# hila-chefer/Transformer-Explainability

Measured on AMD Instinct MI355X. Metric: relevance maps/sec (ViT-B/16 224^2, batch 64 per GPU, generate_LRP transformer_attribution), higher is better.
Workload: dtype f32 (3xbf16 split operands, 6 products, fp32 accumulate)

## Files before the change

### include/te_relprop.h

```cpp
#ifndef TE_RELPROP_H
#define TE_RELPROP_H

#include <stddef.h>
#include <stdint.h>

#ifdef __cplusplus
extern "C" {
#endif

typedef void* te_stream_t;
typedef uint16_t te_bf16_t;

enum {
  TE_OK = 0,
  TE_ERR_INVALID_ARG = -1,
  TE_ERR_WORKSPACE = -2,
  TE_ERR_UNSUPPORTED = -3,
  TE_ERR_NO_DEVICE = -4
};

enum { TE_VARIANT_OURS = 0, TE_VARIANT_LRP = 1, TE_IMPL_SIMPLE = 0x100 };

enum { TE_ROLLOUT_NORMALISE = 1, TE_ROLLOUT_CLS_FIXUP = 2, TE_ROLLOUT_ROW0 = 4 };

// ... 35 lines not shown
                             const float* q, int64_t q_sb, int64_t q_sh, int64_t q_sn,
                             const float* k, int64_t k_sb, int64_t k_sh, int64_t k_sn,
                             const float* Z,
                             float* cam_q, int64_t cq_sb, int64_t cq_sh, int64_t cq_sn,
                             float* cam_k, int64_t ck_sb, int64_t ck_sh, int64_t ck_sn,
                             int64_t B, int64_t H, int64_t N, int64_t D, float out_scale, int variant,
                             void* ws, size_t ws_bytes, te_stream_t stream);

size_t te_add_relprop_workspace_bytes(int64_t B, int64_t n);
int te_add_relprop_f32(const float* R, const float* X0, const float* X1, float* out0, float* out1,
                       int64_t B, int64_t n, int64_t x1_batch_stride, int variant,
                       void* ws, size_t ws_bytes, te_stream_t stream);

size_t te_add_relprop_deferred_workspace_bytes(int64_t B, int64_t n);
int te_add_relprop_deferred_f32(const float* R, const float* X0, const float* X1, float* a, float* b, float* fac,
                                int64_t B, int64_t n, int64_t x1_batch_stride,
                                void* ws, size_t ws_bytes, te_stream_t stream);

size_t te_add_bcast_relprop_workspace_bytes(int64_t B, int64_t H, int64_t N);
int te_add_bcast_relprop_f32(const float* R, const float* X0, const float* mask, float* out0,
                             float* out1, int64_t B, int64_t H, int64_t N, int variant,
                             void* ws, size_t ws_bytes, te_stream_t stream);

int te_add_bcast_relprop_deferred_f32(const float* R, const float* X0, const float* mask, float* a, float* out1,
                                      float* fac, int64_t B, int64_t H, int64_t N,
                                      void* ws, size_t ws_bytes, te_stream_t stream);

int te_clone_relprop_f32(const float* R0, const float* R1, const float* R2, const float* X,
                         float* out, int64_t n, te_stream_t stream);

int te_clone_relprop_scaled_f32(const float* R0, const float* s0, int64_t s0_stride,
                                const float* R1, const float* s1, int64_t s1_stride,
                                const float* R2, const float* s2, int64_t s2_stride,
                                const float* X, float* out, int64_t B, int64_t n, te_stream_t stream);

int te_index_select_relprop_f32(const float* R, const float* X, float* out,
                                int64_t B, int64_t N, int64_t C, int64_t index, te_stream_t stream);

int te_gradcam_headmean_f32(const float* grad, const float* cam, float* out,
                            int64_t B, int64_t H, int64_t N, te_stream_t stream);

size_t te_rollout_workspace_bytes(int64_t L, int64_t B, int64_t N);
size_t te_rollout_row0_workspace_bytes(int64_t B, int64_t N);
int te_rollout_f32(const float* cams, int64_t L, int64_t start_layer, int64_t B, int64_t N,
                   int flags, float* joint, void* ws, size_t ws_bytes, te_stream_t stream);

#define TE_X6_TILE_AUTO 0
#define TE_X6_TILE_128 1
#define TE_X6_TILE_256 2
#define TE_X6_TILE_128x128 3
#define TE_X6_TEST_DROP_HANDOVER 0x200
#define TE_X6_WHOLE_TILES 0x10000
#define TE_X6_TEST_SMALL_GRID 0x4000
#define TE_X6_X_PLANES_SIGNED 0x20000
#define TE_X6_TILE_Z_SHIFT 10
#define TE_X6_TILE_C_SHIFT 12
#define TE_X6_PHASE_SPLIT 4
#define TE_X6_PHASE_Z 8
#define TE_X6_PHASE_C 16
#define TE_X6_PHASE_MASK 28
int te_linear_relprop_x6_supported(int64_t T, int64_t in_f, int64_t out_f);
size_t te_linear_relprop_x6_workspace_bytes(int64_t T, int64_t in_f, int64_t out_f);
size_t te_linear_x6_weight_planes_bytes(int64_t in_f, int64_t out_f);
size_t te_linear_x6_planes_bytes(int64_t rows, int64_t K);
int te_linear_x6_prepare_weights_f32(const float* W, int64_t in_f, int64_t out_f, void* planes, size_t planes_bytes,
                                     te_stream_t stream);
int te_linear_x6_split_abs_f32(const float* X, int64_t rows, int64_t K, void* planes, size_t planes_bytes,
                               te_stream_t stream);
int te_linear_relprop_x6_f32(const float* R, const float* r_scale, int64_t r_scale_stride, int64_t rows_per_sample,
                             const float* X, const float* W, const void* w_planes, const void* x_planes,
                             const float* Y, const float* bias, float* out,
                             int64_t T, int64_t in_f, int64_t out_f, int flags, unsigned* status, void* ws,
                             size_t ws_bytes, te_stream_t stream);
int te_linear_relprop_x6_check(const void* ws, int64_t T, int64_t in_f, int64_t out_f, te_stream_t stream);

int te_linear_relprop_x6_general_supported(int64_t T, int64_t in_f, int64_t out_f, int variant);
size_t te_linear_x6_weight_planes_lrp_bytes(int64_t in_f, int64_t out_f);
int te_linear_x6_prepare_weights_lrp_f32(const float* W, int64_t in_f, int64_t out_f, void* planes, size_t planes_bytes,
                                         te_stream_t stream);
size_t te_linear_relprop_x6_general_workspace_bytes(int64_t T, int64_t in_f, int64_t out_f, int variant);
int te_linear_relprop_x6_general_f32(const float* R, const float* r_scale, int64_t r_scale_stride, int64_t rows_per_sample,
                                     const float* X, const float* W, const void* w_planes, const void* w_planes_lrp,
                                     const void* x_abs_planes, const float* Y, const float* bias, float* out,
                                     int64_t T, int64_t in_f, int64_t out_f, float alpha, int variant, int flags,
                                     unsigned* status, void* ws, size_t ws_bytes, te_stream_t stream);

int te_gemm_x6_supported(int64_t T, int64_t K, int64_t M);
size_t te_gemm_x6_workspace_bytes(int64_t T, int64_t K, int64_t M);
int te_linear_x6_split_matrix_f32(const float* A, int64_t rows, int64_t K, int transposed, void* planes,
                                  size_t planes_bytes, te_stream_t stream);
int te_gemm_x6_f32(const float* X, const void* x_planes, const void* w_planes, const float* bias, float* out,
                   int64_t T, int64_t K, int64_t M, int flags, unsigned* status, void* ws, size_t ws_bytes,
                   te_stream_t stream);
int te_linear_x6_split_dual_f32(const float* A, int64_t rows, int64_t K, void* planes, void* planes_abs,
                                size_t planes_bytes, te_stream_t stream);
int te_gelu_backward_x6_planes_f32(const float* dy, const float* x, int64_t rows, int64_t K, void* planes,
                                   size_t planes_bytes, te_stream_t stream);
int te_gelu_forward_x6_planes_f32(const float* x, float* y, int64_t rows, int64_t K, void* planes, void* planes_abs,
                                  size_t planes_bytes, te_stream_t stream);

int te_attention_forward_supported(int64_t N, int64_t D);
int te_attention_forward_f32(const float* qkv, float* z_qk, float* attn, float* out, void* out_planes,
                             void* out_abs_planes, size_t planes_bytes, int64_t B, int64_t H, int64_t N, int64_t D,
                             float scale, te_stream_t stream);
int te_attention_backward_f32(const float* d_out, const float* out, const float* qkv, const float* attn, float* d_attn,
                              float* d_qkv, int64_t B, int64_t H, int64_t N, int64_t D, float scale, int need_qk,
                              te_stream_t stream);

int te_attention_strided_supported(int64_t N, int64_t D);
size_t te_attention_backward_strided_workspace_bytes(int64_t B, int64_t H, int64_t N);
int te_attention_forward_strided_f32(const float* q, int64_t q_sb, int64_t q_sh, int64_t q_sn,
                                     const float* k, int64_t k_sb, int64_t k_sh, int64_t k_sn,
                                     const float* v, int64_t v_sb, int64_t v_sh, int64_t v_sn,
                                     const float* mask, float* z_qk, float* x_scaled, float* attn,
                                     float* out, int64_t o_sb, int64_t o_sh, int64_t o_sn,
                                     int64_t B, int64_t H, int64_t N, int64_t D, float scale, te_stream_t stream);
int te_attention_backward_strided_f32(const float* d_out, int64_t do_sb, int64_t do_sh, int64_t do_sn,
                                      const float* out, int64_t o_sb, int64_t o_sh, int64_t o_sn,
                                      const float* q, int64_t q_sb, int64_t q_sh, int64_t q_sn,
                                      const float* k, int64_t k_sb, int64_t k_sh, int64_t k_sn,
                                      const float* v, int64_t v_sb, int64_t v_sh, int64_t v_sn,
                                      const float* attn, float* d_attn,
                                      float* d_q, int64_t dq_sb, int64_t dq_sh, int64_t dq_sn,
                                      float* d_k, int64_t dk_sb, int64_t dk_sh, int64_t dk_sn,
                                      float* d_v, int64_t dv_sb, int64_t dv_sh, int64_t dv_sn,
                                      int64_t B, int64_t H, int64_t N, int64_t D, float scale, int need_qk,
                                      void* ws, size_t ws_bytes, te_stream_t stream);
// ... 239 lines not shown
```

### transformer-explainability_amd/csrc/te_linear_x6.hip

```cpp
#include <algorithm>
#include <cmath>
#include <type_traits>

#include "te_x6.h"

namespace {

constexpr int kRB = 3 * kFrag;
constexpr int kMinFrag = 4;
constexpr int kSpinMillis = 250;
constexpr int kErrWord = 1023;


enum { MODE_Z = 0, MODE_C = 1, MODE_G = 2, MODE_ZI = 3, MODE_Z1 = 4, MODE_CI = 5, MODE_X = 6, MODE_ZS = 7 };

__device__ __forceinline__ float bf16_f32(unsigned b) { return __uint_as_float(b << 16); }

enum { OP_ABS = 0, OP_POS = 1, OP_NEG = 2, OP_ID = 3 };
template <int OP>
__device__ __forceinline__ float apply_op(float x) {
  if constexpr (OP == OP_ID) return x;
  if constexpr (OP == OP_ABS) return __int_as_float(__float_as_int(x) & 0x7fffffff);
  const int b = __float_as_int(x);
  if constexpr (OP == OP_POS) return __int_as_float(b > 0 ? b : 0);
  return __int_as_float(b < 0 ? b : 0);
}

template <int OP, bool TRANSPOSE>
__global__ __launch_bounds__(256) void split_kernel(const float* __restrict__ src, unsigned char* __restrict__ dst,
                                                    int64_t R, int64_t K, int group, int sign,
                                                    unsigned char* __restrict__ dst_abs = nullptr) {
  const int r = threadIdx.x & 31, sl = threadIdx.x >> 5;
  const int64_t rb = blockIdx.x;
  const int64_t ks = (int64_t)blockIdx.y * 8 + sl;
  const int64_t nks = K >> 4;
  if (ks >= nks) return;
  const int64_t row = rb * 32 + r;
  float v[16];
  if (row < R) {
    if constexpr (!TRANSPOSE) {
      const float* s = src + row * K + ks * 16;
#pragma unroll
      for (int c = 0; c < 4; ++c) {
        const f32x4 q = *reinterpret_cast<const f32x4*>(s + 4 * c);
#pragma unroll
        for (int e = 0; e < 4; ++e) v[4 * c + e] = q[e];
      }
    } else {
#pragma unroll
      for (int e = 0; e < 16; ++e) v[e] = src[(ks * 16 + e) * R + row];
    }
  } else {
#pragma unroll
    for (int e = 0; e < 16; ++e) v[e] = 0.0f;
  }
  unsigned p[8][3];
#pragma unroll
  for (int e = 0; e < 8; ++e) split3_pk(apply_op<OP>(v[2 * e]), apply_op<OP>(v[2 * e + 1]), p[e]);
  unsigned char* d = dst + ((rb * nks + ks) * group + sign * 3) * kFrag + r * 16;
#pragma unroll
  for (int q = 0; q < 3; ++q)
#pragma unroll
    for (int kh = 0; kh < 2; ++kh) {
      u32x4 w;
// ... 88 lines not shown
      p[e][0] &= 0x7fff7fffu;
      p[e][1] ^= m & (((p[e][1] & 0x7fff7fffu) + 0x7fff7fffu) & 0x80008000u);
      p[e][2] ^= m & (((p[e][2] & 0x7fff7fffu) + 0x7fff7fffu) & 0x80008000u);
    }
    store(dst_abs + ((rb * nks + ks) * 3) * kFrag + r * 16);
  }
}

__global__ __launch_bounds__(256) void zero_words_kernel(u32x4* __restrict__ p) {
  p[(size_t)blockIdx.x * 256 + threadIdx.x] = u32x4{0u, 0u, 0u, 0u};
}

__device__ __forceinline__ float exact_z(const float* __restrict__ x, const float* __restrict__ w, int64_t K) {
  float z1 = 0.0f, z2 = 0.0f;
  for (int64_t k = 0; k < K; ++k) {
    const float xv = x[k], wv = w[k];
    z1 = fmaf(fmaxf(xv, 0.0f), fmaxf(wv, 0.0f), z1);
    z2 = fmaf(fminf(xv, 0.0f), fminf(wv, 0.0f), z2);
  }
  return z1 + z2;
}

__device__ __forceinline__ float exact_zi(const float* __restrict__ x, const float* __restrict__ w, int64_t K) {
  float z1 = 0.0f, z2 = 0.0f;
  for (int64_t k = 0; k < K; ++k) {
    const float xv = x[k], wv = w[k];
    z1 = fmaf(fmaxf(xv, 0.0f), fminf(wv, 0.0f), z1);
    z2 = fmaf(fminf(xv, 0.0f), fmaxf(wv, 0.0f), z2);
  }
  return z1 + z2;
}

struct X6Params {
  const unsigned char* A;
  const unsigned char* B;
  int64_t a_group_stride;
  int64_t b_rb_stride;
  int nks;
  unsigned char pad0_[20];
  int ntm, ntn;
  int rows_w;
  int t_fast;
  int whole_tiles;
  int pad1_;
  int ncb;
  int64_t T;
  int in_f, out_f;
  float* partial;
  unsigned* flags;
  unsigned* status;
  long long spin_ticks;
  int drop_handover;
  int small_grid;
  int prefer_whole;
  const float* R;
  const float* Y;
  const float* bias;
  const float* X;
  const float* W;
  unsigned char* S;
  const float* rs;
  int64_t rs_stride;
  int rps;
  float* out;
  float scale;
  int accum;
  int x_sign;
};

#if defined(__HIP_DEVICE_COMPILE__)
#define X6_PASS4(a, b, c, d) asm volatile("" : "+v"(a), "+v"(b), "+v"(c), "+v"(d))
#else
#define X6_PASS4(a, b, c, d) (void)0
#endif

__device__ __forceinline__ void glds16(const unsigned char* src, unsigned char* lds_wave_base) {
  __builtin_amdgcn_global_load_lds((const __attribute__((address_space(1))) void*)src,
                                   (__attribute__((address_space(3))) void*)lds_wave_base, 16, 0, 0);
}

constexpr int kStages = 2;
template <int WM>
struct X6Geo {
  static constexpr int NWM = (WM == 1) ? 1 : 2, NWN = (WM == 0) ? 2 : 4, MI = (WM == 0) ? 2 : 4;
  static constexpr int NW = NWM * NWN, THREADS = 64 * NW, WPS = (WM == 0) ? 3 : 2;
  static constexpr int TM = NWM * MI * 32, TT = NWN * 64;
  static constexpr int NPA = 3 * NWM * MI, NPB = 3 * NWN * 2;
  static constexpr int ACC = MI * 2 * 16;
  static constexpr int MAX_SPX = (WM == 2) ? 32 : (WM == 1) ? 64 : 96;
};

template <int WM, int MODE>
struct X6Lds {
  using GEO = X6Geo<WM>;
  static constexpr bool STAGED = (MODE == MODE_Z || MODE == MODE_ZS || MODE == MODE_ZI || MODE == MODE_Z1) && GEO::MI == 4;
  static constexpr int STAGES = kStages * (GEO::NPA + GEO::NPB) * kFrag;
  static constexpr int MAIN = (STAGED && GEO::NW * 16384 > STAGES) ? GEO::NW * 16384 : STAGES;
  static constexpr int TOTAL = MAIN + GEO::NW * 512 + 16;
};

template <int WM, int MODE>
__global__ __launch_bounds__(X6Geo<WM>::THREADS, X6Geo<WM>::WPS) void x6_kernel(const X6Params p) {
  using GEO = X6Geo<WM>;
  constexpr int NW = GEO::NW, NWM = GEO::NWM, NWN = GEO::NWN, MI = GEO::MI;
  constexpr bool SGN = MODE == MODE_ZS;
  constexpr bool Z_ABS = MODE == MODE_Z || SGN;
  constexpr bool IS_Z = (Z_ABS || MODE == MODE_ZI || MODE == MODE_Z1);
  constexpr bool IS_C = (MODE == MODE_C || MODE == MODE_CI);
  constexpr int G = IS_C ? 6 : 3;
  constexpr int NPA = GEO::NPA, NPB = GEO::NPB;
  constexpr int NP = NPA + NPB;
  static_assert(NPA / 3 == NW, "each wave stages one weight-side block");
  constexpr int PBW = NPB / 3 / NW;
  constexpr int STAGE = NP * kFrag;
  constexpr int GROUPS = NPA / G;
  constexpr int LDS_MAIN = X6Lds<WM, MODE>::MAIN;
  extern __shared__ __attribute__((aligned(16))) unsigned char smem[];

  const int lane = threadIdx.x & 63;
  const int wave = __builtin_amdgcn_readfirstlane(threadIdx.x >> 6);
  const int wm = wave / NWN, wn = wave % NWN;
  const int lane16 = lane * 16;

  const int bid = blockIdx.x, spx = gridDim.x >> 3;
  const int xcd = bid & 7, slot = bid >> 3;
  const int nks = p.nks;
  const int tiles = p.ntm * p.ntn;
  const int tx0 = (int)((int64_t)tiles * xcd / 8), tx1 = (int)((int64_t)tiles * (xcd + 1) / 8);
  const int ntx = tx1 - tx0;
  const int64_t iters = (int64_t)ntx * nks;
  auto cut = [&](int s) -> int64_t {
    int64_t b = iters * s / spx;
    const int r = (int)(b % nks);
    if (p.whole_tiles) return (2 * r < nks) ? b - r : b + (nks - r);
    if (r < kMinFrag) b -= r;
    else if (nks - r < kMinFrag) b += nks - r;
    return b;
  };
  const int64_t ib = cut(slot), ie = cut(slot + 1);
  if (ib >= ie) return;
  const int f_tile = (int)(ib / nks), kb = (int)(ib - (int64_t)f_tile * nks);
  const int l_tile = (int)((ie - 1) / nks), ke = (int)(ie - (int64_t)l_tile * nks);
  const bool tail = kb > 0;
  const bool head = (ke < nks) && !(f_tile == l_tile && tail);
  const int full0 = tail ? f_tile + 1 : f_tile, full1 = (ke < nks) ? l_tile - 1 : l_tile;
  const int nseq = (head ? 1 : 0) + (full1 >= full0 ? full1 - full0 + 1 : 0) + (tail ? 1 : 0);

  float* my_part = p.partial + (size_t)bid * GEO::THREADS * GEO::ACC;
  const float* in_part = p.partial + (size_t)(bid - 8) * GEO::THREADS * GEO::ACC;

  for (int seq = 0; seq < nseq; ++seq) {
    int tile, k0, k1;
    if (head && seq == 0) {
      tile = l_tile, k0 = 0, k1 = ke;
    } else if (tail && seq == nseq - 1) {
      tile = f_tile, k0 = kb, k1 = (f_tile == l_tile) ? ke : nks;
    } else {
      tile = full0 + seq - (head ? 1 : 0), k0 = 0, k1 = nks;
    }
    tile += tx0;
    int tn, tm;
    if (p.t_fast) {
      tm = tile / p.ntn, tn = tile - tm * p.ntn;
    } else {
      tn = tile / p.ntm, tm = tile - tn * p.ntm;
    }

    const unsigned char* srcA;
    if constexpr (!IS_C)
      srcA = p.A + (int64_t)(tm * GROUPS + wave) * p.a_group_stride + (int64_t)k0 * kRB;
    else
      srcA = p.A + (int64_t)(tm * GROUPS + (wave >> 1)) * p.a_group_stride + (int64_t)k0 * (2 * kRB) + (wave & 1) * kRB;
    const unsigned char* srcB[PBW];
#pragma unroll
    for (int u = 0; u < PBW; ++u) {
      const int cb = min(tn * (GEO::TT / 32) + wave * PBW + u, p.ncb - 1);
      srcB[u] = p.B + (int64_t)cb * p.b_rb_stride + (int64_t)k0 * kRB;
    }
    unsigned char* const ldsA = smem + wave * kRB;
    unsigned char* const ldsB = smem + NPA * kFrag + wave * (PBW * kRB);
    u32x4 breg[SGN ? PBW : 1][3];
    auto stage_in = [&](int stg, int adv) __attribute__((always_inline)) {
      srcA += adv * (G * kFrag);
#pragma unroll
      for (int u = 0; u < PBW; ++u) srcB[u] += adv * kRB;
#pragma unroll
      for (int q = 0; q < 3; ++q) glds16(srcA + q * kFrag + lane16, ldsA + stg * STAGE + q * kFrag);
#pragma unroll
      for (int u = 0; u < PBW; ++u)
#pragma unroll
        for (int q = 0; q < 3; ++q) {
          if constexpr (SGN) breg[u][q] = *reinterpret_cast<const u32x4*>(srcB[u] + q * kFrag + lane16);
          else glds16(srcB[u] + q * kFrag + lane16, ldsB + stg * STAGE + (u * 3 + q) * kFrag);
        }
    };
    auto sign_and_store = [&](int stg) __attribute__((always_inline)) {
#pragma unroll
      for (int u = 0; u < (SGN ? PBW : 0); ++u) {
#pragma unroll
        for (int e = 0; e < 4; ++e) {
          const unsigned m = breg[u][0][e] & 0x80008000u;
          breg[u][0][e] &= 0x7fff7fffu;
          breg[u][1][e] ^= m;
          breg[u][2][e] ^= m;
        }
#pragma unroll
// ... 487 lines not shown
      bool live[2];
#pragma unroll
      for (int ni = 0; ni < 2; ++ni) {
        const int64_t t = ((int64_t)tn * (GEO::TT / 32) + wn * 2 + ni) * 32 + tc;
        live[ni] = t < p.T;
        tt[ni] = live[ni] ? t : p.T - 1;
#pragma unroll
        for (int il = 0; il < MI / 2; ++il) {
          const float* xr = p.X + tt[ni] * p.in_f + (tm * (NWM * MI / 2) + wm * (MI / 2) + il) * 32 + 4 * h;
#pragma unroll
          for (int g = 0; g < 4; ++g) x4[ni][il][g] = *reinterpret_cast<const f32x4*>(xr + 8 * g);
        }
      }
#pragma unroll
      for (int ni = 0; ni < 2; ++ni)
#pragma unroll
        for (int il = 0; il < MI / 2; ++il) {
          float* orow = p.out + tt[ni] * p.in_f + (tm * (NWM * MI / 2) + wm * (MI / 2) + il) * 32 + 4 * h;
#pragma unroll
          for (int g = 0; g < 4; ++g) {
            f32x4 o;
#pragma unroll
            for (int c = 0; c < 4; ++c) {
              const float xv = x4[ni][il][g][c];
              const float xp = fmaxf(xv, 0.0f), xn = fminf(xv, 0.0f);
              if constexpr (MODE == MODE_C)
                o[c] = p.scale * (xp * acc[2 * il][ni][4 * g + c] + xn * acc[2 * il + 1][ni][4 * g + c]);
              else
                o[c] = p.scale * (xp * acc[2 * il + 1][ni][4 * g + c] + xn * acc[2 * il][ni][4 * g + c]);
            }
            if constexpr (MODE == MODE_CI) {
              const f32x4 prev = *reinterpret_cast<const f32x4*>(orow + 8 * g);
#pragma unroll
              for (int c = 0; c < 4; ++c) o[c] = prev[c] + o[c];
            }
            if (live[ni]) *reinterpret_cast<f32x4*>(orow + 8 * g) = o;
          }
        }
    }
    __syncthreads();
  }
}

static_assert(sizeof(X6Params) == 248, "X6Params is the kernel-argument block of x6_kernel");
static_assert(offsetof(X6Params, ntm) == 56 && offsetof(X6Params, ncb) == 80 && offsetof(X6Params, T) == 88 &&
              offsetof(X6Params, partial) == 104 && offsetof(X6Params, R) == 152 && offsetof(X6Params, out) == 224,
              "a field of X6Params moved in the kernel arguments");

inline size_t planes_bytes(int64_t rows, int64_t K) {
  return (size_t)te_ceil_div(rows, 32) * 32 * (size_t)K * 6;
}
inline bool bad_k(int64_t K) { return K < 16 || K % 16; }
constexpr size_t kPartialBytes = (size_t)512 * 256 * 128 * 4;
constexpr double kWholeTileSlack = 1.15;
constexpr size_t kFlagBytes = 65536;
constexpr int kFlagWords = kFlagBytes / 4;
constexpr int kUsedFlagWords = kErrWord + 1;
constexpr int kRulePasses = 2;
constexpr int kGeneralPasses = 8;

struct X6Workspace {
  size_t x_stride, s, s_stride, partial, flags, total;
  unsigned char* x(void* ws, int set) const { return (unsigned char*)ws + set * x_stride; }
  unsigned char* sp(void* ws, int set) const { return (unsigned char*)ws + s + set * s_stride; }
  float* acc(void* ws) const { return (float*)((unsigned char*)ws + partial); }
  unsigned* flag_region(const void* ws, int pass) const { return (unsigned*)((unsigned char*)ws + flags) + (size_t)pass * kFlagWords; }
};
inline X6Workspace x6_workspace(int64_t T, int64_t K, int64_t M, int xsets, int ssets, int passes) {
  X6Workspace l;
  l.x_stride = te_align_up(planes_bytes(T, K), 256);
  l.s_stride = te_align_up(planes_bytes(T, M), 256);
  l.s = xsets * l.x_stride;
  l.partial = l.s + ssets * l.s_stride;
  l.flags = l.partial + kPartialBytes;
  l.total = l.flags + passes * kFlagBytes;
  return l;
}
inline X6Workspace gemm_workspace(int64_t T, int64_t K, int64_t M) { return x6_workspace(T, K, M, 1, 0, 1); }
inline X6Workspace rule_workspace(int64_t T, int64_t in_f, int64_t out_f) { return x6_workspace(T, in_f, out_f, 1, 1, kRulePasses); }
inline X6Workspace general_workspace(int64_t T, int64_t in_f, int64_t out_f) { return x6_workspace(T, in_f, out_f, 2, 2, kGeneralPasses); }

struct X6WeightPlanes { size_t c, total; };
inline X6WeightPlanes weight_planes(int64_t in_f, int64_t out_f) {
  const size_t c = te_align_up(planes_bytes(out_f, in_f), 256);
  return {c, c + te_align_up(2 * planes_bytes(in_f, out_f), 256)};
}
struct X6WeightPlanesLrp { size_t wn, wpT, wnT, total; };
inline X6WeightPlanesLrp weight_planes_lrp(int64_t in_f, int64_t out_f) {
  const size_t za = te_align_up(planes_bytes(out_f, in_f), 256), ca = te_align_up(planes_bytes(in_f, out_f), 256);
  return {za, 2 * za, 2 * za + ca, 2 * za + 2 * ca};
}

constexpr int kTileMask = TE_X6_TILE_128 | TE_X6_TILE_256 | TE_X6_TILE_128x128;
constexpr int kProductFlags = kTileMask | TE_X6_WHOLE_TILES | TE_X6_TEST_DROP_HANDOVER | TE_X6_TEST_SMALL_GRID;
constexpr int kRuleFlags = kProductFlags | TE_X6_PHASE_MASK | TE_X6_X_PLANES_SIGNED | (kTileMask << TE_X6_TILE_Z_SHIFT) | (kTileMask << TE_X6_TILE_C_SHIFT);

inline int pick_wm(int64_t in_f, int64_t out_f) {
  if (out_f % 256 == 0 && in_f % 128 == 0) return 2;
  if (out_f % 128 == 0 && in_f % 64 == 0) return 1;
  return 0;
}

inline long long spin_ticks_for_current_device() {
  static long long cached[64] = {};
  int dev = 0;
  if (hipGetDevice(&dev) != hipSuccess || dev < 0 || dev >= 64) dev = 0;
  if (cached[dev] == 0) {
    int khz = 0;
    if (hipDeviceGetAttribute(&khz, hipDeviceAttributeWallClockRate, dev) != hipSuccess || khz <= 0) khz = 100000;
    cached[dev] = (long long)khz * kSpinMillis;
  }
  return cached[dev];
}

template <int WM, int MODE>
int launch_x6(const X6Params& p, hipStream_t stream) {
  using GEO = X6Geo<WM>;
  constexpr int lds = X6Lds<WM, MODE>::TOTAL;
  static_assert(lds * (WM == 0 ? 3 : WM == 1 ? 2 : 1) <= 160 * 1024, "LDS of the workgroups of one CU");
  static_assert((size_t)8 * GEO::MAX_SPX * GEO::THREADS * GEO::ACC * 4 <= kPartialBytes && 8 * GEO::MAX_SPX < kErrWord, "workspace");
  auto kern = x6_kernel<WM, MODE>;
  hipError_t e = hipFuncSetAttribute(reinterpret_cast<const void*>(kern), hipFuncAttributeMaxDynamicSharedMemorySize, lds);
  if (e != hipSuccess) return (int)e;
  X6Params q = p;
  q.ntm = p.rows_w / GEO::TM;
  q.ntn = (int)te_ceil_div(p.T, GEO::TT);
  const int64_t tiles = (int64_t)q.ntm * q.ntn;
  const int max_spx = p.small_grid ? 2 : GEO::MAX_SPX;
  const int spx = (int)std::min<int64_t>(max_spx, std::max<int64_t>(1, te_ceil_div(tiles, 8)));
  const double r = (double)tiles / (8.0 * spx);
  q.whole_tiles = ((p.prefer_whole || std::ceil(r) <= kWholeTileSlack * r) && !p.small_grid) ? 1 : 0;
  if (!q.status) q.status = q.flags + kErrWord;
  q.spin_ticks = spin_ticks_for_current_device();
  kern<<<dim3(8 * spx), dim3(GEO::THREADS), lds, stream>>>(q);
  return TE_OK;
}

template <int MODE>
int launch_x6_mode(int wm, const X6Params& p, hipStream_t stream) {
  if (wm == 2) return launch_x6<2, MODE>(p, stream);
  if (wm == 1) return launch_x6<1, MODE>(p, stream);
  return launch_x6<0, MODE>(p, stream);
}

inline int choose_geo(int wm_max, int64_t T, int64_t rows_w, int pin, int min_tiles_256 = 256, bool small_ok = false) {
  if (pin == TE_X6_TILE_128) return 1;
  if (pin == TE_X6_TILE_256) return wm_max;
  if (pin == TE_X6_TILE_128x128) return 0;
  const int64_t t256 = te_ceil_div(T, 256);
  if (wm_max == 2 && t256 * (rows_w / 256) >= min_tiles_256) return 2;
  if (small_ok && t256 * (rows_w / 128) < 448) return 0;
  return 1;
}

inline X6Params call_params(int64_t T, float* partial, const float* bias, float* out, unsigned* status, int flags) {
  X6Params p{};
  p.T = T;
  p.ncb = (int)te_ceil_div(T, 32);
  p.partial = partial;
  p.bias = bias;
  p.out = out;
  p.status = status;
  p.drop_handover = (flags & TE_X6_TEST_DROP_HANDOVER) ? 1 : 0;
  p.small_grid = (flags & TE_X6_TEST_SMALL_GRID) ? 1 : 0;
  p.prefer_whole = (flags & TE_X6_WHOLE_TILES) ? 1 : 0;
  return p;
}
inline X6Params rule_params(X6Params p, const float* R, const float* r_scale, int64_t r_scale_stride, int64_t rows_per_sample,
                            const float* X, const float* W, const float* Y) {
  p.R = R;
  p.Y = Y;
  p.X = X;
  p.W = W;
  p.rs = r_scale;
  p.rs_stride = r_scale_stride;
  p.rps = (int)(r_scale ? rows_per_sample : 1);
  return p;
}
inline bool bad_r_scale(const float* r_scale, int64_t rows_per_sample, int64_t T) {
  return r_scale && (rows_per_sample <= 0 || rows_per_sample > 0x7fffffff || T % rows_per_sample);
}

template <int MODE>
int launch_pass(X6Params p, int wm, const unsigned char* A, const unsigned char* B, unsigned char* S, int64_t in_f,
                int64_t out_f, unsigned* flag_region, hipStream_t stream, float scale = 0.0f, int accum = 0, int x_sign = 0) {
  constexpr bool c_like = MODE == MODE_C || MODE == MODE_CI;
  constexpr bool over_out = c_like || MODE == MODE_X;
  p.A = A, p.B = B, p.S = S;
  p.nks = (int)((over_out ? out_f : in_f) / 16);
  p.a_group_stride = (int64_t)p.nks * (c_like ? 2 : 1) * kRB;
  p.b_rb_stride = (int64_t)p.nks * kRB;
  p.rows_w = (int)(c_like ? 2 * in_f : MODE == MODE_X ? in_f : out_f);
  p.in_f = (int)(MODE == MODE_X ? out_f : in_f);
  p.out_f = (int)(MODE == MODE_X ? in_f : out_f);
  p.scale = scale, p.accum = accum, p.x_sign = x_sign;
  p.flags = flag_region;
  return launch_x6_mode<MODE>(wm, p, stream);
}

inline void zero_flag_regions(unsigned* flag_words, int passes, hipStream_t stream) {
  zero_words_kernel<<<dim3(passes * kFlagBytes / 16 / 256), dim3(256), 0, stream>>>(reinterpret_cast<u32x4*>(flag_words));
}

inline int check_producer(bool have_all, bool f32_aligned, bool planes_aligned, int64_t rows, int64_t K, size_t planes_bytes_) {
  if (!have_all || rows < 1) return TE_ERR_INVALID_ARG;
  if (bad_k(K) || !f32_aligned || rows > ((int64_t)1 << 26)) return TE_ERR_UNSUPPORTED;
  if (planes_bytes_ < planes_bytes(rows, K) || !planes_aligned) return TE_ERR_WORKSPACE;
  return TE_OK;
}
inline dim3 producer_grid(int64_t rows, int64_t K) { return dim3((unsigned)te_ceil_div(rows, 32), (unsigned)te_ceil_div(K / 16, 8)); }

}

extern "C" int te_linear_relprop_x6_supported(int64_t T, int64_t in_f, int64_t out_f) {
  return (T >= 1 && in_f >= 128 && out_f >= 128 && pick_wm(in_f, out_f) != 0 && in_f <= (1 << 20) && out_f <= (1 << 20) &&
          T <= (int64_t)1 << 26) ? 1 : 0;
}

// ... 51 lines not shown
extern "C" int te_linear_x6_split_dual_f32(const float* A, int64_t rows, int64_t K, void* planes, void* planes_abs,
                                           size_t planes_bytes_, te_stream_t stream_) {
  const int rc = check_producer(A && planes && planes_abs, te_aligned16(A), te_aligned16(planes) && te_aligned16(planes_abs), rows, K, planes_bytes_);
  if (rc != TE_OK) return rc;
  split_kernel<OP_ID, false><<<producer_grid(rows, K), dim3(256), 0, (hipStream_t)stream_>>>(A, (unsigned char*)planes, rows, K, 3, 0,
                                                                                           (unsigned char*)planes_abs);
  TE_RETURN_IF_LAUNCH_FAILED();
  return TE_OK;
}

extern "C" int te_gelu_backward_x6_planes_f32(const float* dy, const float* x, int64_t rows, int64_t K, void* planes,
                                              size_t planes_bytes_, te_stream_t stream_) {
  const int rc = check_producer(dy && x && planes, te_aligned16(dy) && te_aligned16(x), te_aligned16(planes), rows, K, planes_bytes_);
  if (rc != TE_OK) return rc;
  gelu_split_lds_kernel<SRC_GELU_BWD><<<producer_grid(rows, K), dim3(256), 0, (hipStream_t)stream_>>>(
      dy, x, nullptr, (unsigned char*)planes, nullptr, rows, K);
  TE_RETURN_IF_LAUNCH_FAILED();
  return TE_OK;
}

extern "C" int te_gelu_forward_x6_planes_f32(const float* x, float* y, int64_t rows, int64_t K, void* planes, void* planes_abs,
                                             size_t planes_bytes_, te_stream_t stream_) {
  const int rc = check_producer(x && y && planes, te_aligned16(x) && te_aligned16(y),
                                te_aligned16(planes) && (!planes_abs || te_aligned16(planes_abs)), rows, K, planes_bytes_);
  if (rc != TE_OK) return rc;
  gelu_split_lds_kernel<SRC_GELU_FWD><<<producer_grid(rows, K), dim3(256), 0, (hipStream_t)stream_>>>(
      nullptr, x, y, (unsigned char*)planes, (unsigned char*)planes_abs, rows, K);
  TE_RETURN_IF_LAUNCH_FAILED();
  return TE_OK;
}

extern "C" size_t te_gemm_x6_workspace_bytes(int64_t T, int64_t K, int64_t M) {
  return te_gemm_x6_supported(T, K, M) ? gemm_workspace(T, K, M).total : 0;
}

extern "C" int te_gemm_x6_f32(const float* X, const void* x_planes, const void* w_planes, const float* bias, float* out,
                              int64_t T, int64_t K, int64_t M, int flags, unsigned* status, void* ws, size_t ws_bytes,
                              te_stream_t stream_) {
  if ((!X && !x_planes) || !w_planes || !out) return TE_ERR_INVALID_ARG;
  if ((flags & ~kProductFlags) != 0) return TE_ERR_INVALID_ARG;
  if (!te_gemm_x6_supported(T, K, M)) return TE_ERR_UNSUPPORTED;
  if (!ws || ws_bytes < te_gemm_x6_workspace_bytes(T, K, M) || !te_aligned16(ws)) return TE_ERR_WORKSPACE;
  if ((X && !te_aligned16(X)) || !te_aligned16(out) || !te_aligned16(w_planes) || (bias && !te_aligned16(bias)) ||
      (x_planes && !te_aligned16(x_planes)))
    return TE_ERR_UNSUPPORTED;
  hipStream_t stream = (hipStream_t)stream_;
  const X6Workspace l = gemm_workspace(T, K, M);
  zero_flag_regions(l.flag_region(ws, 0), 1, stream);
  if (!x_planes) {
    int rc = te_linear_x6_split_matrix_f32(X, T, K, 0, l.x(ws, 0), planes_bytes(T, K), stream_);
    if (rc != TE_OK) return rc;
    x_planes = l.x(ws, 0);
  }
  const int wm = choose_geo((M % 256 == 0) ? 2 : 1, T, M, flags & kTileMask, 192, true);
  const int rc = launch_pass<MODE_G>(call_params(T, l.acc(ws), bias, out, status, flags), wm, (const unsigned char*)w_planes,
                                     (const unsigned char*)x_planes, nullptr, K, M, l.flag_region(ws, 0), stream);
  if (rc != TE_OK) return rc;
  TE_RETURN_IF_LAUNCH_FAILED();
  return TE_OK;
}

extern "C" size_t te_linear_relprop_x6_workspace_bytes(int64_t T, int64_t in_f, int64_t out_f) {
  return te_linear_relprop_x6_supported(T, in_f, out_f) ? rule_workspace(T, in_f, out_f).total : 0;
}

extern "C" int te_linear_relprop_x6_f32(const float* R, const float* r_scale, int64_t r_scale_stride,
                                        int64_t rows_per_sample, const float* X, const float* W, const void* w_planes,
                                        const void* x_planes, const float* Y, const float* bias, float* out, int64_t T,
                                        int64_t in_f, int64_t out_f, int flags, unsigned* status, void* ws,
                                        size_t ws_bytes, te_stream_t stream_) {
  if (!R || !X || !W || !w_planes || !Y || !out || T <= 0) return TE_ERR_INVALID_ARG;
  if (!te_linear_relprop_x6_supported(T, in_f, out_f)) return TE_ERR_UNSUPPORTED;
  if (!ws || ws_bytes < te_linear_relprop_x6_workspace_bytes(T, in_f, out_f) || !te_aligned16(ws)) return TE_ERR_WORKSPACE;
  if (!te_aligned16(X) || !te_aligned16(W) || !te_aligned16(R) || !te_aligned16(Y) || !te_aligned16(out) ||
      !te_aligned16(w_planes) || (bias && !te_aligned16(bias)) || (x_planes && !te_aligned16(x_planes)))
    return TE_ERR_UNSUPPORTED;
  if (bad_r_scale(r_scale, rows_per_sample, T)) return TE_ERR_INVALID_ARG;
  if ((flags & ~kRuleFlags) != 0) return TE_ERR_INVALID_ARG;
  const int phases = (flags & TE_X6_PHASE_MASK) ? (flags & TE_X6_PHASE_MASK) : TE_X6_PHASE_MASK;
  hipStream_t stream = (hipStream_t)stream_;
  const X6Workspace l = rule_workspace(T, in_f, out_f);
  unsigned char* Ss = l.sp(ws, 0);
  const unsigned char* wz = (const unsigned char*)w_planes;
  const unsigned char* wc = wz + weight_planes(in_f, out_f).c;

  if (phases & TE_X6_PHASE_SPLIT) zero_flag_regions(l.flag_region(ws, 0), kRulePasses, stream);
  const bool x_signed = (flags & TE_X6_X_PLANES_SIGNED) != 0;
  if (!x_planes) {
    if (phases & TE_X6_PHASE_SPLIT) {
      int rc = x_signed ? te_linear_x6_split_matrix_f32(X, T, in_f, 0, l.x(ws, 0), planes_bytes(T, in_f), stream_)
                        : te_linear_x6_split_abs_f32(X, T, in_f, l.x(ws, 0), planes_bytes(T, in_f), stream_);
      if (rc != TE_OK) return rc;
    }
    x_planes = l.x(ws, 0);
  }
  const int wm_max = pick_wm(in_f, out_f);
  const int pz = (flags >> TE_X6_TILE_Z_SHIFT) & kTileMask, pc = (flags >> TE_X6_TILE_C_SHIFT) & kTileMask;
  const int wm_z = choose_geo(wm_max, T, out_f, pz ? pz : (flags & kTileMask), 256, true);
  const int wm_c = choose_geo(wm_max, T, 2 * in_f, pc ? pc : (flags & kTileMask));
  const X6Params p = rule_params(call_params(T, l.acc(ws), bias, out, status, flags), R, r_scale, r_scale_stride, rows_per_sample,
                                 X, W, Y);
  int rc;
  if (phases & TE_X6_PHASE_Z) {
    rc = x_signed ? launch_pass<MODE_ZS>(p, wm_z, wz, (const unsigned char*)x_planes, Ss, in_f, out_f, l.flag_region(ws, 0), stream, 1.0f)
                  : launch_pass<MODE_Z>(p, wm_z, wz, (const unsigned char*)x_planes, Ss, in_f, out_f, l.flag_region(ws, 0), stream, 1.0f);
    if (rc != TE_OK) return rc;
  }
  if (phases & TE_X6_PHASE_C) {
    rc = launch_pass<MODE_C>(p, wm_c, wc, Ss, Ss, in_f, out_f, l.flag_region(ws, 1), stream, 1.0f);
    if (rc != TE_OK) return rc;
  }
  TE_RETURN_IF_LAUNCH_FAILED();
  return TE_OK;
}

extern "C" int te_linear_relprop_x6_general_supported(int64_t T, int64_t in_f, int64_t out_f, int variant) {
  if (!te_linear_relprop_x6_supported(T, in_f, out_f)) return 0;
  if (variant == TE_VARIANT_LRP) return (in_f % 128 == 0) ? 1 : 0;
  return variant == TE_VARIANT_OURS ? 1 : 0;
}

extern "C" size_t te_linear_x6_weight_planes_lrp_bytes(int64_t in_f, int64_t out_f) {
  return te_linear_relprop_x6_general_supported(1, in_f, out_f, TE_VARIANT_LRP) ? weight_planes_lrp(in_f, out_f).total : 0;
}

extern "C" int te_linear_x6_prepare_weights_lrp_f32(const float* W, int64_t in_f, int64_t out_f, void* planes,
                                                    size_t planes_bytes_, te_stream_t stream_) {
  if (!W || !planes) return TE_ERR_INVALID_ARG;
  if (!te_linear_relprop_x6_general_supported(1, in_f, out_f, TE_VARIANT_LRP) || !te_aligned16(W)) return TE_ERR_UNSUPPORTED;
  if (planes_bytes_ < te_linear_x6_weight_planes_lrp_bytes(in_f, out_f) || !te_aligned16(planes)) return TE_ERR_WORKSPACE;
  hipStream_t stream = (hipStream_t)stream_;
  unsigned char* q = (unsigned char*)planes;
  const X6WeightPlanesLrp wl = weight_planes_lrp(in_f, out_f);
  const dim3 gz = producer_grid(out_f, in_f), gc = producer_grid(in_f, out_f);
  split_kernel<OP_POS, false><<<gz, dim3(256), 0, stream>>>(W, q, out_f, in_f, 3, 0);
  split_kernel<OP_NEG, false><<<gz, dim3(256), 0, stream>>>(W, q + wl.wn, out_f, in_f, 3, 0);
  split_kernel<OP_POS, true><<<gc, dim3(256), 0, stream>>>(W, q + wl.wpT, in_f, out_f, 3, 0);
  split_kernel<OP_NEG, true><<<gc, dim3(256), 0, stream>>>(W, q + wl.wnT, in_f, out_f, 3, 0);
  TE_RETURN_IF_LAUNCH_FAILED();
  return TE_OK;
}

extern "C" size_t te_linear_relprop_x6_general_workspace_bytes(int64_t T, int64_t in_f, int64_t out_f, int variant) {
  return te_linear_relprop_x6_general_supported(T, in_f, out_f, variant) ? general_workspace(T, in_f, out_f).total : 0;
}

extern "C" int te_linear_relprop_x6_general_f32(const float* R, const float* r_scale, int64_t r_scale_stride,
                                                int64_t rows_per_sample, const float* X, const float* W,
                                                const void* w_planes, const void* w_planes_lrp, const void* x_abs_planes,
                                                const float* Y, const float* bias, float* out, int64_t T, int64_t in_f,
                                                int64_t out_f, float alpha, int variant, int flags, unsigned* status,
                                                void* ws, size_t ws_bytes, te_stream_t stream_) {
// ... 23 lines not shown
  int pass = 0;
  int rc;
  if (!lrp) {
    const unsigned char* wz = (const unsigned char*)w_planes;
    const unsigned char* wc = wz + weight_planes(in_f, out_f).c;
    if (!x_abs_planes) {
      rc = te_linear_x6_split_abs_f32(X, T, in_f, Xa, planes_bytes(T, in_f), stream_);
      if (rc != TE_OK) return rc;
      x_abs_planes = Xa;
    }
    const int wm_c = choose_geo(pick_wm(in_f, out_f), T, 2 * in_f, pin);
    rc = launch_pass<MODE_Z>(p, wm_z, wz, (const unsigned char*)x_abs_planes, Sa, in_f, out_f, l.flag_region(ws, pass++), stream);
    if (rc != TE_OK) return rc;
    rc = launch_pass<MODE_C>(p, wm_c, wc, Sa, nullptr, in_f, out_f, l.flag_region(ws, pass++), stream, alpha);
    if (rc != TE_OK) return rc;
    if (beta != 0.0f) {
      rc = launch_pass<MODE_ZI>(p, wm_z, wz, (const unsigned char*)x_abs_planes, Sa, in_f, out_f, l.flag_region(ws, pass++), stream);
      if (rc != TE_OK) return rc;
      rc = launch_pass<MODE_CI>(p, wm_c, wc, Sa, nullptr, in_f, out_f, l.flag_region(ws, pass++), stream, -beta);
      if (rc != TE_OK) return rc;
    }
  } else {
    const X6WeightPlanesLrp wl = weight_planes_lrp(in_f, out_f);
    const unsigned char* Wp = (const unsigned char*)w_planes_lrp;
    const unsigned char* Wn = Wp + wl.wn, *WpT = Wp + wl.wpT, *WnT = Wp + wl.wnT;
    split_kernel<OP_POS, false><<<producer_grid(T, in_f), dim3(256), 0, stream>>>(X, Xa, T, in_f, 3, 0);
    split_kernel<OP_NEG, false><<<producer_grid(T, in_f), dim3(256), 0, stream>>>(X, Xb, T, in_f, 3, 0);
    const int wm_x = choose_geo((in_f % 256 == 0) ? 2 : 1, T, in_f, pin, 192, true);
    auto x_pass = [&](const unsigned char* AT, const unsigned char* S, int sign, float scale, int accum) -> int {
      return launch_pass<MODE_X>(p, wm_x, AT, S, nullptr, in_f, out_f, l.flag_region(ws, pass++), stream, scale, accum, sign);
    };
    for (int half = 0; half < (beta != 0.0f ? 2 : 1); ++half) {
      const unsigned char* w1 = half ? Wn : Wp, *w2 = half ? Wp : Wn, *w1T = half ? WnT : WpT, *w2T = half ? WpT : WnT;
      const float sc = half ? -beta : alpha;
      if (half) {
        pass = 0;
        static_assert(kGeneralPasses >= 5, "four passes per half + the region of the per-call error word");
        zero_flag_regions(l.flag_region(ws, 0), 4, stream);
      }
      rc = launch_pass<MODE_Z1>(p, wm_z, w1, Xa, Sa, in_f, out_f, l.flag_region(ws, pass++), stream);
      if (rc != TE_OK) return rc;
      rc = launch_pass<MODE_Z1>(p, wm_z, w2, Xb, Sb, in_f, out_f, l.flag_region(ws, pass++), stream);
      if (rc != TE_OK) return rc;
      rc = x_pass(w1T, Sa, +1, sc, half);
      if (rc != TE_OK) return rc;
      rc = x_pass(w2T, Sb, -1, sc, 1);
      if (rc != TE_OK) return rc;
    }
  }
  TE_RETURN_IF_LAUNCH_FAILED();
  return TE_OK;
}

extern "C" int te_linear_relprop_x6_check(const void* ws, int64_t T, int64_t in_f, int64_t out_f, te_stream_t stream_) {
  if (!ws || !te_linear_relprop_x6_supported(T, in_f, out_f)) return TE_ERR_INVALID_ARG;
  const X6Workspace l = rule_workspace(T, in_f, out_f);
  unsigned host[kRulePasses][kUsedFlagWords];
  hipError_t e = hipSuccess;
  for (int pass = 0; pass < kRulePasses && e == hipSuccess; ++pass)
    e = hipMemcpyAsync(host[pass], l.flag_region(ws, pass), sizeof(host[pass]), hipMemcpyDeviceToHost, (hipStream_t)stream_);
  if (e == hipSuccess) e = hipStreamSynchronize((hipStream_t)stream_);
  if (e != hipSuccess) return (int)e;
  for (int pass = 0; pass < kRulePasses; ++pass)
    for (int i = 0; i < kUsedFlagWords; ++i)
      if (host[pass][i]) return 1;
  return 0;
}
```

### transformer-explainability_amd/ops.py

```python
from __future__ import annotations

import contextlib
import os
from typing import Optional, Sequence, Tuple

import torch

from . import _lib
from ._lib import (TE_HEADMEAN_CLAMP, TE_HEADMEAN_ROW0, TE_IMPL_SIMPLE, TE_RATIONALE_CLAMP, TE_ROLLOUT_CLS_FIXUP,
                   TE_ROLLOUT_NORMALISE, TE_ROLLOUT_ROW0, TE_VARIANT_LRP, TE_VARIANT_OURS)
from ._lib import (TE_X6_PHASE_C, TE_X6_PHASE_SPLIT, TE_X6_PHASE_Z, TE_X6_TEST_DROP_HANDOVER,
                   TE_X6_TEST_SMALL_GRID, TE_X6_TILE_C_SHIFT, TE_X6_TILE_Z_SHIFT, TE_X6_WHOLE_TILES, TE_X6_X_PLANES_SIGNED)

Tensor = torch.Tensor
_VARIANTS = {"ours": TE_VARIANT_OURS, "lrp": TE_VARIANT_LRP}

FORCE_SIMPLE = False
KERNEL_TIMER = None
_NULL = contextlib.nullcontext()


def _timed(name: str, flops: float = 0.0, nbytes: float = 0.0):
    return _NULL if KERNEL_TIMER is None else KERNEL_TIMER(name, float(flops), float(nbytes))


class Deferred:
    __slots__ = ("t", "scale")

    def __init__(self, t: Tensor, scale: Tensor):
        self.t, self.scale = t, scale

    @property
    def shape(self):
        return self.t.shape

    def materialise(self) -> Tensor:
        return self.t * self.scale.view(-1, *([1] * (self.t.dim() - 1)))


def _split_deferred(x):
    return (x.t, x.scale) if isinstance(x, Deferred) else (x, None)
_checked_device = False


def _variant(v) -> int:
    code = _VARIANTS[v] if isinstance(v, str) else int(v)
    return code | (TE_IMPL_SIMPLE if FORCE_SIMPLE else 0)


DTYPES_MSG = ("relprop kernels take float32 tensors, or bfloat16 operands with float32 relevance, or float64 operands with "
              "float64 relevance, the latter two on the ViT / DeiT and BERT rules of variant 'ours' with alpha = 1")


def _prep(t: Tensor) -> Tensor:
    if t.dtype != torch.float32:
        raise _lib.TeError(f"{DTYPES_MSG}; got {t.dtype} here")
    if not t.is_cuda:
        raise _lib.TeError("relprop kernels need tensors on the MI355X (got a CPU tensor); there is no CPU fallback")
    return t


def _is_bf16(t) -> bool:
    return torch.is_tensor(t) and t.dtype == torch.bfloat16


# ... 2269 lines not shown
```

Baseline: 1037.

## Add dynamic whole-tile claiming and cost-model schedule choice for x6 GEMM passes

Replaces the slack-ratio rule that chose between stream-K and whole-tile scheduling with a step-time cost model comparing lock-step rounds against skewed stream-K time, with margins that depend on the tile shape. When whole tiles are chosen, workgroups now claim tiles dynamically from a per-XCD atomic counter by default, instead of using a fixed static partition. The aim is to cut load imbalance and the overhead of partial-tile handover. In exchange it adds an atomic and a barrier per tile, and it zeroes the flag regions when passes run separately so the counters are reset. A schedule-query API is also exposed.

```diff
diff --git a/include/te_relprop.h b/include/te_relprop.h
--- a/include/te_relprop.h
+++ b/include/te_relprop.h
@@ -111,6 +111,8 @@
 #define TE_X6_TEST_DROP_HANDOVER 0x200
 #define TE_X6_WHOLE_TILES 0x10000
 #define TE_X6_TEST_SMALL_GRID 0x4000
+#define TE_X6_SLACK_RULE 0x100000
+#define TE_X6_STATIC_TILES 0x80000
 #define TE_X6_X_PLANES_SIGNED 0x20000
 #define TE_X6_TILE_Z_SHIFT 10
 #define TE_X6_TILE_C_SHIFT 12
@@ -132,6 +134,13 @@
                              int64_t T, int64_t in_f, int64_t out_f, int flags, unsigned* status, void* ws,
                              size_t ws_bytes, te_stream_t stream);
 int te_linear_relprop_x6_check(const void* ws, int64_t T, int64_t in_f, int64_t out_f, te_stream_t stream);
+#define TE_X6_PASS_Z 0
+#define TE_X6_PASS_C 1
+#define TE_X6_PASS_PRODUCT 2
+#define TE_X6_SCHEDULE_STREAM_K 0
+#define TE_X6_SCHEDULE_WHOLE_STATIC 1
+#define TE_X6_SCHEDULE_WHOLE_CLAIMED 2
+int te_linear_x6_schedule(int64_t T, int64_t in_f, int64_t out_f, int pass, int flags, int* schedule);
 
 int te_linear_relprop_x6_general_supported(int64_t T, int64_t in_f, int64_t out_f, int variant);
 size_t te_linear_x6_weight_planes_lrp_bytes(int64_t in_f, int64_t out_f);
diff --git a/transformer-explainability_amd/csrc/te_linear_x6.hip b/transformer-explainability_amd/csrc/te_linear_x6.hip
--- a/transformer-explainability_amd/csrc/te_linear_x6.hip
+++ b/transformer-explainability_amd/csrc/te_linear_x6.hip
@@ -10,6 +10,7 @@
 constexpr int kMinFrag = 4;
 constexpr int kSpinMillis = 250;
 constexpr int kErrWord = 1023;
+constexpr int kClaimWord = 1024, kClaimStride = 32;
 
 
 enum { MODE_Z = 0, MODE_C = 1, MODE_G = 2, MODE_ZI = 3, MODE_Z1 = 4, MODE_CI = 5, MODE_X = 6, MODE_ZS = 7 };
@@ -204,7 +205,7 @@
   long long spin_ticks;
   int drop_handover;
   int small_grid;
-  int prefer_whole;
+  int sched_flags;
   const float* R;
   const float* Y;
   const float* bias;
@@ -289,8 +290,10 @@
     else if (nks - r < kMinFrag) b += nks - r;
     return b;
   };
+  const bool claim = p.whole_tiles == 2;
+  unsigned* const claim_ctr = p.flags + kClaimWord + xcd * kClaimStride;
   const int64_t ib = cut(slot), ie = cut(slot + 1);
-  if (ib >= ie) return;
+  if (!claim && ib >= ie) return;
   const int f_tile = (int)(ib / nks), kb = (int)(ib - (int64_t)f_tile * nks);
   const int l_tile = (int)((ie - 1) / nks), ke = (int)(ie - (int64_t)l_tile * nks);
   const bool tail = kb > 0;
@@ -301,9 +304,16 @@
   float* my_part = p.partial + (size_t)bid * GEO::THREADS * GEO::ACC;
   const float* in_part = p.partial + (size_t)(bid - 8) * GEO::THREADS * GEO::ACC;
 
-  for (int seq = 0; seq < nseq; ++seq) {
+  for (int seq = 0; claim || seq < nseq; ++seq) {
     int tile, k0, k1;
-    if (head && seq == 0) {
+    if (claim) {
+      unsigned* const claimed = reinterpret_cast<unsigned*>(smem + X6Lds<WM, MODE>::MAIN + NW * 512) + 1;
+      if (threadIdx.x == 0) *claimed = __hip_atomic_fetch_add(claim_ctr, 1u, __ATOMIC_RELAXED, __HIP_MEMORY_SCOPE_AGENT);
+      __syncthreads();
+      tile = (int)__builtin_amdgcn_readfirstlane(*claimed);
+      if (tile >= ntx) break;
+      k0 = 0, k1 = nks;
+    } else if (head && seq == 0) {
       tile = l_tile, k0 = 0, k1 = ke;
     } else if (tail && seq == nseq - 1) {
       tile = f_tile, k0 = kb, k1 = (f_tile == l_tile) ? ke : nks;
@@ -897,7 +907,6 @@
 }
 inline bool bad_k(int64_t K) { return K < 16 || K % 16; }
 constexpr size_t kPartialBytes = (size_t)512 * 256 * 128 * 4;
-constexpr double kWholeTileSlack = 1.15;
 constexpr size_t kFlagBytes = 65536;
 constexpr int kFlagWords = kFlagBytes / 4;
 constexpr int kUsedFlagWords = kErrWord + 1;
@@ -937,7 +946,8 @@
 }
 
 constexpr int kTileMask = TE_X6_TILE_128 | TE_X6_TILE_256 | TE_X6_TILE_128x128;
-constexpr int kProductFlags = kTileMask | TE_X6_WHOLE_TILES | TE_X6_TEST_DROP_HANDOVER | TE_X6_TEST_SMALL_GRID;
+constexpr int kScheduleFlags = TE_X6_WHOLE_TILES | TE_X6_SLACK_RULE | TE_X6_STATIC_TILES;
+constexpr int kProductFlags = kTileMask | kScheduleFlags | TE_X6_TEST_DROP_HANDOVER | TE_X6_TEST_SMALL_GRID;
 constexpr int kRuleFlags = kProductFlags | TE_X6_PHASE_MASK | TE_X6_X_PLANES_SIGNED | (kTileMask << TE_X6_TILE_Z_SHIFT) | (kTileMask << TE_X6_TILE_C_SHIFT);
 
 inline int pick_wm(int64_t in_f, int64_t out_f) {
@@ -958,9 +968,43 @@
   return cached[dev];
 }
 
+constexpr double kStepLockShort = 2.27, kStepLockLong = 2.00;
+constexpr double kStepSkewShort = 2.60, kStepSkewLong = 2.32;
+constexpr int kShortSteps = 48, kLongSteps = 144;
+constexpr double kWallMargin = 0.05, kWallMarginPacked = 0.20;
+constexpr double kWholeTileSlack = 1.15;
+inline double step_time(int nks, double t_short, double t_long) {
+  if (nks <= kShortSteps) return t_short;
+  if (nks >= kLongSteps) return t_long;
+  return t_short + (t_long - t_short) * (nks - kShortSteps) / (kLongSteps - kShortSteps);
+}
+struct X6Schedule { int ntm, ntn, tiles, spx, whole_tiles; };
+inline X6Schedule plan_x6(int wm, int64_t T, int rows_w, int nks, int small_grid, int sched_flags) {
+  const int tm = (wm == 2) ? 256 : 128, tt = (wm == 0) ? 128 : 256, geo_max_spx = (wm == 2) ? 32 : (wm == 1) ? 64 : 96;
+  X6Schedule s;
+  s.ntm = rows_w / tm;
+  s.ntn = (int)te_ceil_div(T, tt);
+  const int64_t tiles = (int64_t)s.ntm * s.ntn;
+  s.tiles = (int)tiles;
+  const int max_spx = small_grid ? 2 : geo_max_spx;
+  s.spx = (int)std::min<int64_t>(max_spx, std::max<int64_t>(1, te_ceil_div(tiles, 8)));
+  const double r = (double)tiles / (8.0 * s.spx), rounds = std::ceil(r);
+  bool whole;
+  if (sched_flags & TE_X6_WHOLE_TILES) whole = true;
+  else if (small_grid) whole = false;
+  else if (sched_flags & TE_X6_SLACK_RULE) whole = rounds <= kWholeTileSlack * r;
+  else {
+    const double margin = ((sched_flags & kTileMask) == TE_X6_TILE_256) ? kWallMarginPacked : kWallMargin;
+    whole = rounds * step_time(nks, kStepLockShort, kStepLockLong) <= (1.0 + margin) * r * step_time(nks, kStepSkewShort, kStepSkewLong);
+  }
+  s.whole_tiles = !whole ? 0 : (sched_flags & TE_X6_STATIC_TILES) ? 1 : 2;
+  return s;
+}
+
 template <int WM, int MODE>
 int launch_x6(const X6Params& p, hipStream_t stream) {
   using GEO = X6Geo<WM>;
+  static_assert(GEO::TM == ((WM == 2) ? 256 : 128) && GEO::TT == ((WM == 0) ? 128 : 256), "plan_x6 restates the tile sizes");
   constexpr int lds = X6Lds<WM, MODE>::TOTAL;
   static_assert(lds * (WM == 0 ? 3 : WM == 1 ? 2 : 1) <= 160 * 1024, "LDS of the workgroups of one CU");
   static_assert((size_t)8 * GEO::MAX_SPX * GEO::THREADS * GEO::ACC * 4 <= kPartialBytes && 8 * GEO::MAX_SPX < kErrWord, "workspace");
@@ -968,16 +1012,14 @@
   hipError_t e = hipFuncSetAttribute(reinterpret_cast<const void*>(kern), hipFuncAttributeMaxDynamicSharedMemorySize, lds);
   if (e != hipSuccess) return (int)e;
   X6Params q = p;
-  q.ntm = p.rows_w / GEO::TM;
-  q.ntn = (int)te_ceil_div(p.T, GEO::TT);
-  const int64_t tiles = (int64_t)q.ntm * q.ntn;
-  const int max_spx = p.small_grid ? 2 : GEO::MAX_SPX;
-  const int spx = (int)std::min<int64_t>(max_spx, std::max<int64_t>(1, te_ceil_div(tiles, 8)));
-  const double r = (double)tiles / (8.0 * spx);
-  q.whole_tiles = ((p.prefer_whole || std::ceil(r) <= kWholeTileSlack * r) && !p.small_grid) ? 1 : 0;
+  const X6Schedule s = plan_x6(WM, p.T, p.rows_w, p.nks, p.small_grid, p.sched_flags);
+  static_assert(GEO::MAX_SPX == ((WM == 2) ? 32 : (WM == 1) ? 64 : 96), "plan_x6 restates the grid limit");
+  q.ntm = s.ntm;
+  q.ntn = s.ntn;
+  q.whole_tiles = s.whole_tiles;
   if (!q.status) q.status = q.flags + kErrWord;
   q.spin_ticks = spin_ticks_for_current_device();
-  kern<<<dim3(8 * spx), dim3(GEO::THREADS), lds, stream>>>(q);
+  kern<<<dim3(8 * s.spx), dim3(GEO::THREADS), lds, stream>>>(q);
   return TE_OK;
 }
 
@@ -997,6 +1039,15 @@
   if (small_ok && t256 * (rows_w / 128) < 448) return 0;
   return 1;
 }
+inline int geo_z(int64_t T, int64_t in_f, int64_t out_f, int flags) {
+  const int pz = (flags >> TE_X6_TILE_Z_SHIFT) & kTileMask;
+  return choose_geo(pick_wm(in_f, out_f), T, out_f, pz ? pz : (flags & kTileMask), 256, true);
+}
+inline int geo_c(int64_t T, int64_t in_f, int64_t out_f, int flags) {
+  const int pc = (flags >> TE_X6_TILE_C_SHIFT) & kTileMask;
+  return choose_geo(pick_wm(in_f, out_f), T, 2 * in_f, pc ? pc : (flags & kTileMask));
+}
+inline int geo_product(int64_t T, int64_t M, int flags) { return choose_geo((M % 256 == 0) ? 2 : 1, T, M, flags & kTileMask, 192, true); }
 
 inline X6Params call_params(int64_t T, float* partial, const float* bias, float* out, unsigned* status, int flags) {
   X6Params p{};
@@ -1008,7 +1059,7 @@
   p.status = status;
   p.drop_handover = (flags & TE_X6_TEST_DROP_HANDOVER) ? 1 : 0;
   p.small_grid = (flags & TE_X6_TEST_SMALL_GRID) ? 1 : 0;
-  p.prefer_whole = (flags & TE_X6_WHOLE_TILES) ? 1 : 0;
+  p.sched_flags = flags & (kScheduleFlags | kTileMask);
   return p;
 }
 inline X6Params rule_params(X6Params p, const float* R, const float* r_scale, int64_t r_scale_stride, int64_t rows_per_sample,
@@ -1166,7 +1217,7 @@
     if (rc != TE_OK) return rc;
     x_planes = l.x(ws, 0);
   }
-  const int wm = choose_geo((M % 256 == 0) ? 2 : 1, T, M, flags & kTileMask, 192, true);
+  const int wm = geo_product(T, M, flags);
   const int rc = launch_pass<MODE_G>(call_params(T, l.acc(ws), bias, out, status, flags), wm, (const unsigned char*)w_planes,
                                      (const unsigned char*)x_planes, nullptr, K, M, l.flag_region(ws, 0), stream);
   if (rc != TE_OK) return rc;
@@ -1199,6 +1250,10 @@
   const unsigned char* wc = wz + weight_planes(in_f, out_f).c;
 
   if (phases & TE_X6_PHASE_SPLIT) zero_flag_regions(l.flag_region(ws, 0), kRulePasses, stream);
+  else {
+    const int first = (phases & TE_X6_PHASE_Z) ? 0 : 1, last = (phases & TE_X6_PHASE_C) ? 1 : 0;
+    zero_flag_regions(l.flag_region(ws, first), last - first + 1, stream);
+  }
   const bool x_signed = (flags & TE_X6_X_PLANES_SIGNED) != 0;
   if (!x_planes) {
     if (phases & TE_X6_PHASE_SPLIT) {
@@ -1208,10 +1263,7 @@
     }
     x_planes = l.x(ws, 0);
   }
-  const int wm_max = pick_wm(in_f, out_f);
-  const int pz = (flags >> TE_X6_TILE_Z_SHIFT) & kTileMask, pc = (flags >> TE_X6_TILE_C_SHIFT) & kTileMask;
-  const int wm_z = choose_geo(wm_max, T, out_f, pz ? pz : (flags & kTileMask), 256, true);
-  const int wm_c = choose_geo(wm_max, T, 2 * in_f, pc ? pc : (flags & kTileMask));
+  const int wm_z = geo_z(T, in_f, out_f, flags), wm_c = geo_c(T, in_f, out_f, flags);
   const X6Params p = rule_params(call_params(T, l.acc(ws), bias, out, status, flags), R, r_scale, r_scale_stride, rows_per_sample,
                                  X, W, Y);
   int rc;
@@ -1341,6 +1393,23 @@
   return TE_OK;
 }
 
+extern "C" int te_linear_x6_schedule(int64_t T, int64_t in_f, int64_t out_f, int pass, int flags, int* schedule) {
+  if (!schedule) return TE_ERR_INVALID_ARG;
+  const bool product = pass == TE_X6_PASS_PRODUCT;
+  if (pass != TE_X6_PASS_Z && pass != TE_X6_PASS_C && !product) return TE_ERR_INVALID_ARG;
+  if ((flags & ~(product ? kProductFlags : kRuleFlags)) != 0) return TE_ERR_INVALID_ARG;
+  if (!(product ? te_gemm_x6_supported(T, in_f, out_f) : te_linear_relprop_x6_supported(T, in_f, out_f))) return TE_ERR_UNSUPPORTED;
+  const bool c = pass == TE_X6_PASS_C;
+  const int wm = product ? geo_product(T, out_f, flags) : c ? geo_c(T, in_f, out_f, flags) : geo_z(T, in_f, out_f, flags);
+  const X6Schedule s = plan_x6(wm, T, (int)(c ? 2 * in_f : out_f), (int)((c ? out_f : in_f) / 16),
+                               (flags & TE_X6_TEST_SMALL_GRID) ? 1 : 0, flags & (kScheduleFlags | kTileMask));
+  schedule[0] = wm == 2 ? TE_X6_TILE_256 : wm == 1 ? TE_X6_TILE_128 : TE_X6_TILE_128x128;
+  schedule[1] = s.whole_tiles;
+  schedule[2] = 8 * s.spx;
+  schedule[3] = s.tiles;
+  return TE_OK;
+}
+
 extern "C" int te_linear_relprop_x6_check(const void* ws, int64_t T, int64_t in_f, int64_t out_f, te_stream_t stream_) {
   if (!ws || !te_linear_relprop_x6_supported(T, in_f, out_f)) return TE_ERR_INVALID_ARG;
   const X6Workspace l = rule_workspace(T, in_f, out_f);
diff --git a/transformer-explainability_amd/ops.py b/transformer-explainability_amd/ops.py
--- a/transformer-explainability_amd/ops.py
+++ b/transformer-explainability_amd/ops.py
@@ -11,6 +11,8 @@
                    TE_ROLLOUT_NORMALISE, TE_ROLLOUT_ROW0, TE_VARIANT_LRP, TE_VARIANT_OURS)
 from ._lib import (TE_X6_PHASE_C, TE_X6_PHASE_SPLIT, TE_X6_PHASE_Z, TE_X6_TEST_DROP_HANDOVER,
                    TE_X6_TEST_SMALL_GRID, TE_X6_TILE_C_SHIFT, TE_X6_TILE_Z_SHIFT, TE_X6_WHOLE_TILES, TE_X6_X_PLANES_SIGNED)
+from ._lib import (TE_X6_PASS_C, TE_X6_PASS_PRODUCT, TE_X6_PASS_Z, TE_X6_SCHEDULE_STREAM_K,
+                   TE_X6_SCHEDULE_WHOLE_CLAIMED, TE_X6_SCHEDULE_WHOLE_STATIC, TE_X6_SLACK_RULE, TE_X6_STATIC_TILES)
 
 Tensor = torch.Tensor
 _VARIANTS = {"ours": TE_VARIANT_OURS, "lrp": TE_VARIANT_LRP}
```

Result: faster. 1050, median of 6 (+1.3%).
